# AOADMM-DataFusionFramework/Matlab-Code

Hardware: AMD Instinct MI355X
Metric: AO-ADMM outer iters/sec (+ mode-1 MTTKRP GFLOP/s), 2000^3 rank-20 CP (higher is better)
Workload: dtype f32

## Files before the change

matlab-code_amd/csrc/contract.hip:

```cpp
#include "contract.h"
#include "device_utils.h"
#include "small_dev.h"

#include <algorithm>
#include <cstdlib>

namespace aoadmm {

typedef float f32x4 __attribute__((ext_vector_type(4)));
typedef double f64x2 __attribute__((ext_vector_type(2)));
typedef double f64x4 __attribute__((ext_vector_type(4)));

static constexpr int kTileRows = 128;
static constexpr int kGroup = 8;

struct KArgs {
  const void* X;
  const void* frag;
  void* T;
  int64_t tiles_per_batch, ntiles, batch_stride, M, ld, C, Cg, trows;
  int groups_per_chunk, R;
  int flush_every;
};

typedef float f32x2 __attribute__((ext_vector_type(2)));

__global__ void pack_frag16_f32(const double* __restrict__ F, int64_t ldF, int64_t C, int R, int NT, int EX,
                                int64_t Cg, float* __restrict__ frag) {
  const int64_t idx = (int64_t)blockIdx.x * blockDim.x + threadIdx.x;
  const int64_t nmain = (int64_t)NT * Cg * 128;
  if (idx < nmain) {
    const int kk = idx & 1;
    const int lane = (idx >> 1) & 63;
    const int64_t g = (idx >> 7) % Cg;
    const int nt = (int)((idx >> 7) / Cg);
    const int64_t c = 8 * g + 4 * kk + (lane >> 4);
    const int r = 16 * nt + (lane & 15);
    frag[idx] = (c < C && r < R) ? (float)F[c + ldF * r] : 0.f;
  } else if (EX && idx < nmain + Cg * 32) {
    const int64_t j = idx - nmain;
    const int e = j & 3, q = (j >> 2) & 3, kk = (j >> 4) & 1;
    const int64_t g = j >> 5;
    const int64_t c = 8 * g + 4 * kk + q;
    const int r = 16 * NT + e;
    frag[idx] = (c < C && r < R) ? (float)F[c + ldF * r] : 0.f;
  }
}

__device__ __forceinline__ float quarter_sum4(float a, float b, float c, float d) {
  const auto ab = __builtin_amdgcn_permlane16_swap(__float_as_uint(a), __float_as_uint(b), false, false);
  const auto cd = __builtin_amdgcn_permlane16_swap(__float_as_uint(c), __float_as_uint(d), false, false);
  const float s_ab = __uint_as_float(ab[0]) + __uint_as_float(ab[1]);
  const float s_cd = __uint_as_float(cd[0]) + __uint_as_float(cd[1]);
  const auto x = __builtin_amdgcn_permlane32_swap(__float_as_uint(s_ab), __float_as_uint(s_cd), false, false);
  return __uint_as_float(x[0]) + __uint_as_float(x[1]);
}

constexpr int kFlushEvery = 3;
template <int NT, bool EX, bool L2 = false>
__global__ __launch_bounds__(256, NT <= 2 ? 2 : 1) void contract16_f32(KArgs a) {
  static_assert(!L2 || NT == 1, "two-level accumulation exists for one 16-column tile (R <= 20)");
  const int lane = threadIdx.x & 63;
  const int64_t wt = (int64_t)blockIdx.x * 4 + (threadIdx.x >> 6);
  if (wt >= a.ntiles) return;
  const int chunk = blockIdx.y;
  const int64_t b = wt / a.tiles_per_batch;
  const int64_t m0 = (wt - b * a.tiles_per_batch) * kTileRows;
  const int r16 = lane & 15, q = lane >> 4;
  int64_t row0 = m0 + 4 * r16, row1 = m0 + 64 + 4 * r16;
  if (row0 >= a.M) row0 = m0;
  if (row1 >= a.M) row1 = m0;
  const int64_t g0 = (int64_t)chunk * a.groups_per_chunk;
  int64_t g1 = g0 + a.groups_per_chunk;
  if (g1 > a.Cg) g1 = a.Cg;
  const int64_t gfull = (a.C / kGroup < g1) ? a.C / kGroup : g1;
  const float* X = reinterpret_cast<const float*>(a.X) + b * a.batch_stride;
  const float* xp0 = X + row0 + (kGroup * g0 + q) * a.ld;
  const float* xp1 = X + row1 + (kGroup * g0 + q) * a.ld;
  const int64_t ld4 = 4 * a.ld;
  const f32x2* fp = reinterpret_cast<const f32x2*>(a.frag) + g0 * 64 + lane;
  const int64_t fnt = a.Cg * 64;
  const f32x4* fe = reinterpret_cast<const f32x4*>(reinterpret_cast<const f32x2*>(a.frag) + (int64_t)NT * a.Cg * 64) + g0 * 8 + q;

  f32x4 acc[NT][2][4];
  f32x2 accE[2][4][2];
#define AO_PKFMA_LO(ACC, X2, E2) asm("v_pk_fma_f32 %0, %1, %2, %0 op_sel:[0,0,0] op_sel_hi:[0,1,1]" : "+v"(ACC) : "v"(X2), "v"(E2));
#define AO_PKFMA_HI(ACC, X2, E2) asm("v_pk_fma_f32 %0, %1, %2, %0 op_sel:[1,0,0] op_sel_hi:[1,1,1]" : "+v"(ACC) : "v"(X2), "v"(E2));
#pragma unroll
  for (int h = 0; h < 2; ++h)
#pragma unroll
    for (int v = 0; v < 4; ++v) {
      accE[h][v][0] = f32x2{0.f, 0.f};
      accE[h][v][1] = f32x2{0.f, 0.f};
#pragma unroll
      for (int nt = 0; nt < NT; ++nt) acc[nt][h][v] = f32x4{0.f, 0.f, 0.f, 0.f};
    }

  extern __shared__ __attribute__((aligned(16))) float t_lds[];
  double* l2 = reinterpret_cast<double*>(t_lds) + (threadIdx.x >> 6) * 2048 + lane;
  double accE2[2][4];
  if (L2) {
#pragma unroll
    for (int k = 0; k < 32; ++k) l2[k * 64] = 0.0;
#pragma unroll
    for (int h = 0; h < 2; ++h)
#pragma unroll
      for (int v = 0; v < 4; ++v) accE2[h][v] = 0.0;
  }
#define AO_FLUSH()                                                                                   \
  {                                                                                                  \
    _Pragma("unroll") for (int h = 0; h < 2; ++h) {                                                  \
      _Pragma("unroll") for (int vb = 0; vb < 4; vb += 2) {                                          \
        _Pragma("unroll") for (int v = vb; v < vb + 2; ++v)                                          \
          _Pragma("unroll") for (int i = 0; i < 4; ++i) {                                            \
            l2[((h * 4 + v) * 4 + i) * 64] += (double)acc[0][h][v][i];                               \
            acc[0][h][v][i] = 0.f;                                                                   \
          }                                                                                          \
        __builtin_amdgcn_sched_barrier(0);                                                           \
      }                                                                                              \
    }                                                                                                \
    if (EX) {       \
      _Pragma("unroll") for (int h = 0; h < 2; ++h)                                                  \
        _Pragma("unroll") for (int v = 0; v < 4; ++v) {                                              \
          accE2[h][v] += (double)quarter_sum4(accE[h][v][0][0], accE[h][v][0][1], accE[h][v][1][0], accE[h][v][1][1]); \
          accE[h][v][0] = f32x2{0.f, 0.f};                                                           \
          accE[h][v][1] = f32x2{0.f, 0.f};                                                           \
        }                                                                                            \
    }                                                                                                \
  }
  f32x4 x0[4], x1[4], x2[4], e0[2], e1[2], e2[2];
  f32x2 f0[NT], f1[NT], f2[NT];
  const int64_t ng = gfull > g0 ? gfull - g0 : 0;
  const int64_t gstep = kGroup * a.ld;
#define AO_LOAD1(XS, GI, S)                                                                          \
  XS[S] = __builtin_nontemporal_load(reinterpret_cast<const f32x4*>((((S) & 1) ? xp1 : xp0) + (GI) * gstep + ((S) >> 1) * ld4));
#define AO_LOADF(FS, ES, GI)                                                                         \
  {                                                                                                  \
    _Pragma("unroll") for (int nt = 0; nt < NT; ++nt) FS[nt] = fp[(GI) * 64 + nt * fnt];            \
    if (EX) { ES[0] = fe[(GI) * 8]; ES[1] = fe[(GI) * 8 + 4]; }                                      \
  }
#define AO_LOAD_STAGE(XS, FS, ES, GI)                                                                \
  { AO_LOAD1(XS, GI, 0) AO_LOAD1(XS, GI, 1) AO_LOAD1(XS, GI, 2) AO_LOAD1(XS, GI, 3) AO_LOADF(FS, ES, GI) }
#define AO_FMA_S(XS, FS, ES, S)                                                                      \
  {                                                                                                  \
    _Pragma("unroll") for (int v = 0; v < 4; ++v) {                                                  \
      _Pragma("unroll") for (int nt = 0; nt < NT; ++nt)                                              \
        acc[nt][(S) & 1][v] = __builtin_amdgcn_mfma_f32_16x16x4f32(XS[S][v], FS[nt][(S) >> 1], acc[nt][(S) & 1][v], 0, 0, 0); \
    }                                                                                                \
    if (EX) {       \
      const f32x2 xlo_ = __builtin_shufflevector(XS[S], XS[S], 0, 1), xhi_ = __builtin_shufflevector(XS[S], XS[S], 2, 3); \
      const f32x2 ea_ = __builtin_shufflevector(ES[(S) >> 1], ES[(S) >> 1], 0, 1);                   \
      const f32x2 eb_ = __builtin_shufflevector(ES[(S) >> 1], ES[(S) >> 1], 2, 3);                   \
      AO_PKFMA_LO(accE[(S) & 1][0][0], xlo_, ea_) AO_PKFMA_LO(accE[(S) & 1][0][1], xlo_, eb_)        \
      AO_PKFMA_HI(accE[(S) & 1][1][0], xlo_, ea_) AO_PKFMA_HI(accE[(S) & 1][1][1], xlo_, eb_)        \
      AO_PKFMA_LO(accE[(S) & 1][2][0], xhi_, ea_) AO_PKFMA_LO(accE[(S) & 1][2][1], xhi_, eb_)        \
      AO_PKFMA_HI(accE[(S) & 1][3][0], xhi_, ea_) AO_PKFMA_HI(accE[(S) & 1][3][1], xhi_, eb_)        \
    }                                                                                                \
  }
// ... 746 lines not shown
    return;
  }
  AO_REQUIRE(prec == AOADMM_PREC_F32 || prec == AOADMM_PREC_F64, "bad precision id %d", prec);
  AO_REQUIRE(pl.tprec == prec, "contraction plan and tensor precision disagree");
  if (pl.lead) {
    AO_REQUIRE(prec == AOADMM_PREC_F32, "leading-mode contraction exists for fp32 tensors only");
    launch_contract_lead(X, pl, F, ldF, frag_ws, T, s, ev0, ev1);
    return;
  }
  const int64_t Cg = cdiv(pl.C, kGroup);
  KArgs a;
  a.X = X; a.frag = frag_ws; a.T = T;
  a.tiles_per_batch = cdiv(pl.M, tile_rows(prec));
  a.ntiles = pl.nbatch * a.tiles_per_batch;
  a.batch_stride = pl.batch_stride; a.M = pl.M; a.ld = pl.ld; a.C = pl.C; a.Cg = Cg;
  a.trows = pl.trows();
  a.groups_per_chunk = (int)cdiv(Cg, pl.nchunk);
  a.R = pl.R;
  AO_REQUIRE(a.ntiles > 0 && pl.C > 0, "empty contraction");
  dim3 grid((unsigned)cdiv(a.ntiles, 4), (unsigned)pl.nchunk);
  AO_REQUIRE(cdiv(a.ntiles, 4) < (int64_t)2147483647, "tensor too large for one launch");
  if (prec == AOADMM_PREC_F32) {
    AO_REQUIRE(pl.ld % 4 == 0 && pl.M % 4 == 0 && pl.batch_stride % 4 == 0, "f32 layout must be padded to 4");
    const int rem = pl.R % 16;
    const bool ex = pl.R > 16 && rem >= 1 && rem <= 4;
    const int nt16 = ex ? pl.R / 16 : (pl.R + 15) / 16;
    const int64_t total = (int64_t)nt16 * Cg * 128 + (ex ? Cg * 32 : 0);
    pack_frag16_f32<<<(unsigned)cdiv(total, 256), 256, 0, s>>>(F, ldF, pl.C, pl.R, nt16, ex ? 1 : 0, Cg, (float*)frag_ws);
    AO_KERNEL_CHECK();
    size_t tsh = (size_t)4 * kTileRows * pl.R * sizeof(float);
    a.flush_every = kFlushEvery;
    if (nt16 == 1) tsh = (size_t)4 * 16384;
#define AO_GO(K) { if (tsh > 65536) ensure_dynamic_lds(reinterpret_cast<const void*>(K), (int)tsh); if (ev0) AO_HIP(hipEventRecord(ev0, s)); K<<<grid, 256, tsh, s>>>(a); }
    if (nt16 == 1 && !ex) AO_GO((contract16_f32<1, false, true>))
    else if (nt16 == 1) AO_GO((contract16_f32<1, true, true>))
    else if (nt16 == 2 && !ex) AO_GO((contract16_f32<2, false>))
    else if (nt16 == 2) AO_GO((contract16_f32<2, true>))
    else if (nt16 == 3 && !ex) AO_GO((contract16_f32<3, false>))
    else if (nt16 == 3) AO_GO((contract16_f32<3, true>))
    else if (nt16 == 4) AO_GO((contract16_f32<4, false>))
    else throw Error(AOADMM_ERR_UNSUPPORTED, "rank > 64 not supported");
#undef AO_GO
  } else {
    AO_REQUIRE(pl.ld % 2 == 0 && pl.M % 2 == 0 && pl.batch_stride % 2 == 0, "f64 layout must be padded to 2");
    const int rem = pl.R % 16;
    const bool ex = pl.R > 16 && rem >= 1 && rem <= 4;
    const int nt16 = ex ? pl.R / 16 : (pl.R + 15) / 16;
    const int64_t total = (int64_t)nt16 * Cg * 128 + (ex ? Cg * 32 : 0);
    pack_frag_f64<<<(unsigned)cdiv(total, 256), 256, 0, s>>>(F, ldF, pl.C, pl.R, nt16, ex ? 1 : 0, Cg, (double*)frag_ws);
    AO_KERNEL_CHECK();
    const size_t tsh = (size_t)4 * kTileRows64 * pl.R * sizeof(double);
#define AO_GO(K) { if (tsh > 65536) ensure_dynamic_lds(reinterpret_cast<const void*>(K), (int)tsh); if (ev0) AO_HIP(hipEventRecord(ev0, s)); K<<<grid, 256, tsh, s>>>(a); }
    if (nt16 == 1 && !ex) AO_GO((contract_f64<1, false>))
    else if (nt16 == 1) AO_GO((contract_f64<1, true>))
    else if (nt16 == 2 && !ex) AO_GO((contract_f64<2, false>))
    else if (nt16 == 2) AO_GO((contract_f64<2, true>))
    else if (nt16 == 3 && !ex) AO_GO((contract_f64<3, false>))
    else if (nt16 == 3) AO_GO((contract_f64<3, true>))
    else if (nt16 == 4) AO_GO((contract_f64<4, false>))
    else throw Error(AOADMM_ERR_UNSUPPORTED, "rank > 64 not supported");
#undef AO_GO
  }
  if (ev1) AO_HIP(hipEventRecord(ev1, s));
  AO_KERNEL_CHECK();
}

__global__ void factor_rowmajor_k(const double* __restrict__ F, int64_t ldF, int64_t rows, int R,
                                  double* __restrict__ Ft) {
  const int64_t idx = (int64_t)blockIdx.x * blockDim.x + threadIdx.x;
  if (idx >= rows * R) return;
  const int r = (int)(idx / rows);
  const int64_t a = idx - (int64_t)r * rows;
  Ft[a * R + r] = F[a + ldF * r];
}
static void factor_rowmajor(const double* F, int64_t ldF, int64_t rows, int R, double* Ft, hipStream_t s) {
  factor_rowmajor_k<<<(unsigned)cdiv(rows * R, 256), 256, 0, s>>>(F, ldF, rows, R, Ft);
  AO_KERNEL_CHECK();
}

template <typename TT, int VEC> struct TVec;
template <> struct TVec<float, 4> { typedef float type __attribute__((ext_vector_type(4))); };
template <> struct TVec<float, 1> { typedef float type; };
template <> struct TVec<double, 2> { typedef double type __attribute__((ext_vector_type(2))); };
template <> struct TVec<double, 1> { typedef double type; };
template <typename TT, int VEC>
__device__ __forceinline__ void fma_vec(double (&acc)[VEC], const TT* __restrict__ tp, const double* __restrict__ fp) {
  typedef typename TVec<TT, VEC>::type V;
  const V tv = __builtin_nontemporal_load(reinterpret_cast<const V*>(tp));
  if constexpr (VEC == 1) {
    acc[0] += (double)tv * fp[0];
  } else {
#pragma unroll
    for (int v = 0; v < VEC; ++v) acc[v] += (double)tv[v] * fp[v];
  }
}

template <typename TT, int VEC>
struct RVec {
  typename TVec<TT, VEC>::type t;
  double f[VEC];
  __device__ __forceinline__ void load(const TT* __restrict__ tp, const double* __restrict__ fp) {
    t = __builtin_nontemporal_load(reinterpret_cast<const typename TVec<TT, VEC>::type*>(tp));
#pragma unroll
    for (int v = 0; v < VEC; ++v) f[v] = fp[v];
  }
  __device__ __forceinline__ void fma(double (&acc)[VEC]) const {
    if constexpr (VEC == 1) {
      acc[0] += (double)t * f[0];
    } else {
#pragma unroll
      for (int v = 0; v < VEC; ++v) acc[v] += (double)t[v] * f[v];
    }
  }
};

template <typename TT, int VEC>
__global__ void reduce_inner_k(const TT* __restrict__ T, int nchunk, int64_t trows, int64_t A, int64_t Apad, int R,
                               const double* __restrict__ FaT, double scale, double* __restrict__ out,
                               int64_t ldOut, int rowmajor, int has_sys, SysBuild sys) {
  extern __shared__ double sh[];
  if (has_sys && blockIdx.x == 0) { sys_build_rider(sys); return; }
  const int64_t b = (int64_t)blockIdx.x - has_sys;
  const int t = threadIdx.x;
  const int64_t n = A * R, step = (int64_t)blockDim.x * VEC;
  double s0[VEC], s1[VEC], s2[VEC], s3[VEC];
#pragma unroll
  for (int v = 0; v < VEC; ++v) { s0[v] = 0; s1[v] = 0; s2[v] = 0; s3[v] = 0; }
  for (int ch = 0; ch < nchunk; ++ch) {
    const TT* Tb = T + ((int64_t)ch * trows + Apad * b) * R;
    int64_t e = (int64_t)t * VEC;
    for (; e + 3 * step < n; e += 4 * step) {
      RVec<TT, VEC> q0, q1, q2, q3;
      q0.load(Tb + e, FaT + e);
      q1.load(Tb + e + step, FaT + e + step);
      q2.load(Tb + e + 2 * step, FaT + e + 2 * step);
      q3.load(Tb + e + 3 * step, FaT + e + 3 * step);
      __builtin_amdgcn_sched_barrier(0);
      q0.fma(s0); q1.fma(s1); q2.fma(s2); q3.fma(s3);
    }
    for (; e < n; e += step) fma_vec<TT, VEC>(s0, Tb + e, FaT + e);
  }
#pragma unroll
  for (int v = 0; v < VEC; ++v) sh[t * VEC + v] = (s0[v] + s1[v]) + (s2[v] + s3[v]);
  __syncthreads();
  if (t < R) {
    const int nA = blockDim.x * VEC / R;
    double tot = 0.0;
    for (int i = 0; i < nA; ++i) tot += sh[i * R + t];
    if (rowmajor) out[b * R + t] = scale * tot;
    else out[b + ldOut * t] = scale * tot;
  }
}

template <typename TT, int VEC>
__global__ void reduce_inner2_k(const TT* __restrict__ T, int nchunk, int64_t trows, int64_t A, int64_t Apad, int64_t B,
                                int R, const double* __restrict__ FaT, double scale, double* __restrict__ out,
                                int64_t ldOut, int rowmajor, int has_sys, SysBuild sys) {
  extern __shared__ double sh[];
  if (has_sys && blockIdx.x == 0) { sys_build_rider(sys); return; }
  const int64_t b0 = 2 * ((int64_t)blockIdx.x - has_sys);
  const bool two = b0 + 1 < B;
  const int64_t b1 = two ? b0 + 1 : b0;
  const int t = threadIdx.x;
  const int64_t n = A * R, step = (int64_t)blockDim.x * VEC;
  double a0[VEC], a1[VEC], c0[VEC], c1[VEC];
#pragma unroll
  for (int v = 0; v < VEC; ++v) { a0[v] = 0; a1[v] = 0; c0[v] = 0; c1[v] = 0; }
  for (int ch = 0; ch < nchunk; ++ch) {
    const TT* Ta = T + ((int64_t)ch * trows + Apad * b0) * R;
    const TT* Tc = T + ((int64_t)ch * trows + Apad * b1) * R;
    int64_t e = (int64_t)t * VEC;
    for (; e + step < n; e += 2 * step) {
      RVec<TT, VEC> q0, q1, p0, p1;
      q0.load(Ta + e, FaT + e);
      q1.load(Ta + e + step, FaT + e + step);
      p0.t = __builtin_nontemporal_load(reinterpret_cast<const typename TVec<TT, VEC>::type*>(Tc + e));
      p1.t = __builtin_nontemporal_load(reinterpret_cast<const typename TVec<TT, VEC>::type*>(Tc + e + step));
      __builtin_amdgcn_sched_barrier(0);
#pragma unroll
      for (int v = 0; v < VEC; ++v) { p0.f[v] = q0.f[v]; p1.f[v] = q1.f[v]; }
      q0.fma(a0); q1.fma(a1); p0.fma(c0); p1.fma(c1);
    }
    for (; e < n; e += step) {
      RVec<TT, VEC> q0, p0;
      q0.load(Ta + e, FaT + e);
      p0.t = __builtin_nontemporal_load(reinterpret_cast<const typename TVec<TT, VEC>::type*>(Tc + e));
#pragma unroll
      for (int v = 0; v < VEC; ++v) p0.f[v] = q0.f[v];
      q0.fma(a0); p0.fma(c0);
    }
  }
  const int nt = blockDim.x * VEC;
#pragma unroll
  for (int v = 0; v < VEC; ++v) { sh[t * VEC + v] = a0[v] + a1[v]; sh[nt + t * VEC + v] = c0[v] + c1[v]; }
  __syncthreads();
  if (t < 2 * R) {
    const int which = t / R, r = t % R;
    if (which == 0 || two) {
      const int nA = nt / R;
      double tot = 0.0;
      for (int i = 0; i < nA; ++i) tot += sh[which * nt + i * R + r];
      const int64_t b = which ? b1 : b0;
      if (rowmajor) out[b * R + r] = scale * tot;
      else out[b + ldOut * r] = scale * tot;
    }
  }
}

size_t reduce_factor_scratch_bytes(int64_t rows, int R) { return (size_t)rows * R * sizeof(double); }

template <typename TT, int VEC>
static void launch_inner_t(const void* T, int nchunk, int64_t trows, int64_t A, int64_t Apad, int64_t B, int R,
                           const double* FaT, double scale, double* out, int64_t ldOut, hipStream_t s, int rowmajor,
                           const SysBuild* sys) {
  const int hs = sys ? 1 : 0;
  const SysBuild sb = sys ? *sys : SysBuild();
  const int rq = R / VEC;
  int threads = 256 / rq * rq;
  if (threads < rq) threads = rq;
  if (threads * VEC < R) threads = (R + VEC - 1) / VEC;
  if (B >= 1024 && 2 * R <= threads) {
    reduce_inner2_k<TT, VEC><<<(unsigned)((B + 1) / 2 + hs), threads, (size_t)2 * threads * VEC * sizeof(double), s>>>(
        (const TT*)T, nchunk, trows, A, Apad, B, R, FaT, scale, out, ldOut, rowmajor, hs, sb);
    return;
  }
  reduce_inner_k<TT, VEC><<<(unsigned)(B + hs), threads, (size_t)threads * VEC * sizeof(double), s>>>(
      (const TT*)T, nchunk, trows, A, Apad, R, FaT, scale, out, ldOut, rowmajor, hs, sb);
}

static bool sys_can_ride(const SysBuild* sys, int threads_min = 64) {
  return sys != nullptr && sys->R >= 1 && sys->R <= kSysRiderMaxR && threads_min >= 64;
}

bool launch_reduce_inner(const void* T, int tprec, int nchunk, int64_t trows, int64_t A, int64_t Apad,
                         int64_t B, int R, const double* Fa, int64_t ldFa, double scale,
                         double* out, int64_t ldOut, double* ft_scratch, hipStream_t s, const double* FaT,
                         int rowmajor_out, const SysBuild* sys) {
  AO_REQUIRE((int64_t)B < 2147483647ll, "reduce_inner: too many output rows for one launch");
  {
    const int vec = tprec == AOADMM_PREC_F32 ? (R % 4 == 0 ? 4 : 1) : (R % 2 == 0 ? 2 : 1);
    const int rq = R / vec;
    int threads = 256 / rq * rq;
    if (threads < rq) threads = rq;
    if (threads * vec < R) threads = (R + vec - 1) / vec;
    if (!sys_can_ride(sys, threads)) sys = nullptr;
  }
  if (FaT) ft_scratch = const_cast<double*>(FaT);
  else factor_rowmajor(Fa, ldFa, A, R, ft_scratch, s);
  if (tprec == AOADMM_PREC_F32) {
    if (R % 4 == 0) launch_inner_t<float, 4>(T, nchunk, trows, A, Apad, B, R, ft_scratch, scale, out, ldOut, s, rowmajor_out, sys);
    else launch_inner_t<float, 1>(T, nchunk, trows, A, Apad, B, R, ft_scratch, scale, out, ldOut, s, rowmajor_out, sys);
  } else {
    if (R % 2 == 0) launch_inner_t<double, 2>(T, nchunk, trows, A, Apad, B, R, ft_scratch, scale, out, ldOut, s, rowmajor_out, sys);
    else launch_inner_t<double, 1>(T, nchunk, trows, A, Apad, B, R, ft_scratch, scale, out, ldOut, s, rowmajor_out, sys);
  }
  AO_KERNEL_CHECK();
  return sys != nullptr;
}

static void outer_geometry(int64_t A, int64_t B, int R, int vec, int& TA, int64_t& nblkA, int& SB) {
  const int rq = (R + vec - 1) / vec;
  TA = 256 / rq;
  if (TA < 1) TA = 1;
  nblkA = cdiv(A, TA);
  int64_t sb = cdiv(2048, nblkA);
  if (sb > 64) sb = 64;
  if (sb > B) sb = B;
  if (sb < 1) sb = 1;
  SB = (int)sb;
}
static int outer_vec(int tprec, int R) {
  if (tprec == AOADMM_PREC_F32) return R % 4 == 0 ? 4 : 1;
  return R % 2 == 0 ? 2 : 1;
}

size_t reduce_outer_scratch_bytes(int64_t A, int64_t B, int R) {
  size_t worst = 0;
  for (int vec : {1, 2, 4}) {
    int TA, SB; int64_t nb;
    outer_geometry(A, B, R, vec, TA, nb, SB);
    worst = std::max(worst, (size_t)SB * A * R * sizeof(double));
  }
  return worst;
}

template <typename TT, int VEC>
__global__ void reduce_outer_k(const TT* __restrict__ T, int nchunk, int64_t trows, int64_t A,
                               int64_t Apad, int64_t B, int R, int TA, const double* __restrict__ FbT,
                               double* __restrict__ part, int has_sys, SysBuild sys) {
  if (has_sys && blockIdx.x == 0) {
    if (blockIdx.y == 0) sys_build_rider(sys);
    return;
  }
  const int t = threadIdx.x;
  const int rq = R / VEC;
  const int al = t / rq, r = (t - al * rq) * VEC;
  const int64_t a = ((int64_t)blockIdx.x - has_sys) * TA + al;
  const int SB = gridDim.y, sb = blockIdx.y;
  const int64_t bper = (B + SB - 1) / SB;
  const int64_t b0 = sb * bper;
  int64_t b1 = b0 + bper;
  if (b1 > B) b1 = B;
  if (al >= TA || a >= A) return;
  const int64_t bs = Apad * R;
  double s0[VEC], s1[VEC], s2[VEC], s3[VEC];
#pragma unroll
  for (int v = 0; v < VEC; ++v) { s0[v] = 0; s1[v] = 0; s2[v] = 0; s3[v] = 0; }
  for (int ch = 0; ch < nchunk; ++ch) {
    const TT* Tc = T + (int64_t)ch * trows * R + a * R + r;
    const double* Fr = FbT + r;
    int64_t b = b0;
    for (; b + 3 < b1; b += 4) {
      RVec<TT, VEC> q0, q1, q2, q3;
      q0.load(Tc + bs * b, Fr + b * R);
      q1.load(Tc + bs * (b + 1), Fr + (b + 1) * R);
      q2.load(Tc + bs * (b + 2), Fr + (b + 2) * R);
      q3.load(Tc + bs * (b + 3), Fr + (b + 3) * R);
      __builtin_amdgcn_sched_barrier(0);
      q0.fma(s0); q1.fma(s1); q2.fma(s2); q3.fma(s3);
    }
    for (; b < b1; ++b) fma_vec<TT, VEC>(s0, Tc + bs * b, Fr + b * R);
  }
#pragma unroll
  for (int v = 0; v < VEC; ++v) part[((int64_t)sb * A + a) * R + r + v] = (s0[v] + s1[v]) + (s2[v] + s3[v]);
}

__global__ void reduce_outer_fin(const double* __restrict__ part, int SB, int64_t A, int R, double scale,
                                 double* __restrict__ out, int64_t ldOut, int rowmajor) {
  int64_t idx = (int64_t)blockIdx.x * blockDim.x + threadIdx.x;
  if (idx >= A * R) return;
  const int64_t a = idx / R;
  const int r = (int)(idx - a * R);
  double t0 = 0.0, t1 = 0.0;
  int s = 0;
  const int64_t ar = A * R;
  for (; s + 7 < SB; s += 8) {
    const double v0 = part[(int64_t)s * ar + idx], v1 = part[(int64_t)(s + 1) * ar + idx];
    const double v2 = part[(int64_t)(s + 2) * ar + idx], v3 = part[(int64_t)(s + 3) * ar + idx];
    const double v4 = part[(int64_t)(s + 4) * ar + idx], v5 = part[(int64_t)(s + 5) * ar + idx];
    const double v6 = part[(int64_t)(s + 6) * ar + idx], v7 = part[(int64_t)(s + 7) * ar + idx];
    t0 += v0; t1 += v1; t0 += v2; t1 += v3; t0 += v4; t1 += v5; t0 += v6; t1 += v7;
  }
  for (; s + 1 < SB; s += 2) {
    t0 += part[(int64_t)s * ar + idx];
    t1 += part[(int64_t)(s + 1) * ar + idx];
  }
  if (s < SB) t0 += part[(int64_t)s * ar + idx];
  if (rowmajor) out[idx] = scale * (t0 + t1);
  else out[a + ldOut * r] = scale * (t0 + t1);
}

template <typename TT, int VEC>
static void launch_outer_t(const void* T, int nchunk, int64_t trows, int64_t A, int64_t Apad, int64_t B, int R,
                           const double* FbT, double* scratch, int& SB, hipStream_t s, const SysBuild* sys) {
  int TA; int64_t nb;
  outer_geometry(A, B, R, VEC, TA, nb, SB);
  int threads = TA * (R / VEC);
  threads = (threads + 63) / 64 * 64;
  const int hs = sys ? 1 : 0;
  reduce_outer_k<TT, VEC><<<dim3((unsigned)(nb + hs), (unsigned)SB), threads, 0, s>>>((const TT*)T, nchunk, trows, A, Apad, B,
                                                                                    R, TA, FbT, scratch, hs, sys ? *sys : SysBuild());
}

bool launch_reduce_outer(const void* T, int tprec, int nchunk, int64_t trows, int64_t A, int64_t Apad,
                         int64_t B, int R, const double* Fb, int64_t ldFb, double scale,
                         double* out, int64_t ldOut, double* scratch, double* ft_scratch, hipStream_t s,
                         const double* FbT, int rowmajor_out, const SysBuild* sys) {
  if (!sys_can_ride(sys)) sys = nullptr;
  if (FbT) ft_scratch = const_cast<double*>(FbT);
  else factor_rowmajor(Fb, ldFb, B, R, ft_scratch, s);
  int SB = 1;
  const int vec = outer_vec(tprec, R);
  if (tprec == AOADMM_PREC_F32) {
    if (vec == 4) launch_outer_t<float, 4>(T, nchunk, trows, A, Apad, B, R, ft_scratch, scratch, SB, s, sys);
    else launch_outer_t<float, 1>(T, nchunk, trows, A, Apad, B, R, ft_scratch, scratch, SB, s, sys);
  } else {
    if (vec == 2) launch_outer_t<double, 2>(T, nchunk, trows, A, Apad, B, R, ft_scratch, scratch, SB, s, sys);
    else launch_outer_t<double, 1>(T, nchunk, trows, A, Apad, B, R, ft_scratch, scratch, SB, s, sys);
  }
  AO_KERNEL_CHECK();
  reduce_outer_fin<<<(unsigned)cdiv(A * R, 256), 256, 0, s>>>(scratch, SB, A, R, scale, out, ldOut, rowmajor_out);
  AO_KERNEL_CHECK();
  return sys != nullptr;
}

template <typename TT, int RMAX>
__global__ __launch_bounds__(256) void small_mttkrp_k(SmallMttkrp a, int has_sys, SysBuild sys) {
  extern __shared__ double sf[];
  if (has_sys && blockIdx.x == 0) { sys_build_rider(sys); return; }
  const int row = (int)blockIdx.x - has_sys;
  const int R = a.R, Na = a.Na, Nb = a.Nb;
  double* fa = sf;
  double* fb = sf + (size_t)Na * R;
  double* red = fb + (size_t)(Nb > 0 ? Nb : 1) * R;
  for (int e = threadIdx.x; e < Na * R; e += 256) { const int i = e / R, r = e - i * R; fa[e] = a.Fa[i + a.lda * r]; }
  for (int e = threadIdx.x; e < Nb * R; e += 256) { const int i = e / R, r = e - i * R; fb[e] = a.Fb ? a.Fb[i + a.ldb * r] : 1.0; }
  __syncthreads();
  const TT* X = reinterpret_cast<const TT*>(a.X) + (int64_t)row * a.sn;
  double acc[RMAX];
#pragma unroll
  for (int r = 0; r < RMAX; ++r) acc[r] = 0.0;
  const int npairs = Na * Nb;
  for (int p = threadIdx.x; p < npairs; p += 256) {
    const int ia = p % Na, ib = p / Na;
    const double x = (double)X[(int64_t)ia * a.sa + (int64_t)ib * a.sb];
#pragma unroll
    for (int r = 0; r < RMAX; ++r)
      if (r < R) acc[r] += x * (fa[ia * R + r] * fb[ib * R + r]);
  }
  const int lane = threadIdx.x & 63, w = threadIdx.x >> 6;
#pragma unroll
  for (int r = 0; r < RMAX; ++r) {
    const double v = wave_sum(acc[r]);
    if (lane == 0) red[w * RMAX + r] = v;
  }
  __syncthreads();
  if ((int)threadIdx.x < R) {
    const int r = threadIdx.x;
    const double tot = (red[r] + red[RMAX + r]) + (red[2 * RMAX + r] + red[3 * RMAX + r]);
    a.out[row + a.ldOut * r] = a.scale * tot;
  }
}

bool small_mttkrp_ok(int64_t elems, int nd, const int64_t* dims, int R) {
  const bool off = getenv("AOADMM_NO_SMALL_MTTKRP") != nullptr;
  if (off || elems > kSmallMttkrpElems || !(nd == 2 || nd == 3) || R > 16) return false;
  int64_t sum = 0;
  for (int i = 0; i < nd; ++i) sum += dims[i];
  return (size_t)(sum * R + 64) * sizeof(double) <= 40 * 1024;
}

bool small_mttkrp(const SmallMttkrp& a, int prec, int64_t rows, hipStream_t s, const SysBuild* sys) {
  if (!sys_can_ride(sys)) sys = nullptr;
  const int hs = sys ? 1 : 0;
  const SysBuild sb = sys ? *sys : SysBuild();
  AO_REQUIRE(a.R >= 1 && a.R <= 16 && rows >= 1 && a.Na >= 1 && a.Nb >= 1, "small_mttkrp: bad sizes");
  const int rmax = a.R <= 4 ? 4 : (a.R <= 8 ? 8 : 16);
  const size_t lds = ((size_t)(a.Na + a.Nb) * a.R + 4 * rmax) * sizeof(double);
  AO_REQUIRE(lds <= 48 * 1024, "small_mttkrp: factors do not fit LDS");
#define AO_SM(TT, RM) small_mttkrp_k<TT, RM><<<(unsigned)(rows + hs), 256, lds, s>>>(a, hs, sb)
  if (prec == AOADMM_PREC_F32) { if (rmax == 4) AO_SM(float, 4); else if (rmax == 8) AO_SM(float, 8); else AO_SM(float, 16); }
  else { if (rmax == 4) AO_SM(double, 4); else if (rmax == 8) AO_SM(double, 8); else AO_SM(double, 16); }
#undef AO_SM
  AO_KERNEL_CHECK();
  return sys != nullptr;
}

template <typename TT>
__global__ void t_to_colmajor_k(const TT* __restrict__ T, int nchunk, int64_t trows, int64_t A, int R,
                                double scale, double* __restrict__ out, int64_t ldOut) {
  int64_t idx = (int64_t)blockIdx.x * blockDim.x + threadIdx.x;
  if (idx >= A * R) return;
  const int64_t a = idx / R;
  const int r = (int)(idx - a * R);
  double tot = 0.0;
  for (int ch = 0; ch < nchunk; ++ch) tot += (double)T[(int64_t)ch * trows * R + idx];
  out[a + ldOut * r] = scale * tot;
}

void launch_t_to_colmajor(const void* T, int tprec, int nchunk, int64_t trows, int64_t A, int R, double scale,
                          double* out, int64_t ldOut, hipStream_t s) {
  const unsigned nb = (unsigned)cdiv(A * R, 256);
  if (tprec == AOADMM_PREC_F32) t_to_colmajor_k<float><<<nb, 256, 0, s>>>((const float*)T, nchunk, trows, A, R, scale, out, ldOut);
  else t_to_colmajor_k<double><<<nb, 256, 0, s>>>((const double*)T, nchunk, trows, A, R, scale, out, ldOut);
  AO_KERNEL_CHECK();
}

}
```

Baseline: 127.6.

## Generalize inner reduction to NB rows and retile outer reduction with thread groups

The inner reduction kernel now processes NB=4 output rows per block instead of 2, sharing each factor-row load across more T rows, and is chosen based on CU count. The outer reduction is reworked: fixed 256-thread blocks hold multiple B-range groups reduced through LDS, two A rows are handled per thread, and the split count is sized from occupancy-derived resident blocks. The aim is more factor reuse and better bandwidth use in the partial contractions, at the cost of extra registers, LDS and occupancy queries on the host.

```diff
diff --git a/matlab-code_amd/csrc/contract.hip b/matlab-code_amd/csrc/contract.hip
--- a/matlab-code_amd/csrc/contract.hip
+++ b/matlab-code_amd/csrc/contract.hip
@@ -4,6 +4,7 @@
 
 #include <algorithm>
 #include <cstdlib>
+#include <mutex>
 
 namespace aoadmm {
 
@@ -1056,59 +1057,85 @@
   }
 }
 
-template <typename TT, int VEC>
-__global__ void reduce_inner2_k(const TT* __restrict__ T, int nchunk, int64_t trows, int64_t A, int64_t Apad, int64_t B,
-                                int R, const double* __restrict__ FaT, double scale, double* __restrict__ out,
-                                int64_t ldOut, int rowmajor, int has_sys, SysBuild sys) {
+template <typename TT, int VEC, int NB>
+__global__ void reduce_innerN_k(const TT* __restrict__ T, int nchunk, int64_t trows, int64_t A,
+                                int64_t Apad, int64_t B, int R, const double* __restrict__ FaT, double scale,
+                                double* __restrict__ out, int64_t ldOut, int rowmajor, int has_sys, SysBuild sys) {
+  typedef typename TVec<TT, VEC>::type V;
   extern __shared__ double sh[];
   if (has_sys && blockIdx.x == 0) { sys_build_rider(sys); return; }
-  const int64_t b0 = 2 * ((int64_t)blockIdx.x - has_sys);
-  const bool two = b0 + 1 < B;
-  const int64_t b1 = two ? b0 + 1 : b0;
+  const int64_t bf = NB * ((int64_t)blockIdx.x - has_sys);
   const int t = threadIdx.x;
   const int64_t n = A * R, step = (int64_t)blockDim.x * VEC;
-  double a0[VEC], a1[VEC], c0[VEC], c1[VEC];
-#pragma unroll
-  for (int v = 0; v < VEC; ++v) { a0[v] = 0; a1[v] = 0; c0[v] = 0; c1[v] = 0; }
+  double acc[NB][VEC];
+#pragma unroll
+  for (int j = 0; j < NB; ++j)
+#pragma unroll
+    for (int v = 0; v < VEC; ++v) acc[j][v] = 0;
   for (int ch = 0; ch < nchunk; ++ch) {
-    const TT* Ta = T + ((int64_t)ch * trows + Apad * b0) * R;
-    const TT* Tc = T + ((int64_t)ch * trows + Apad * b1) * R;
+    const TT* Tb[NB];
+#pragma unroll
+    for (int j = 0; j < NB; ++j) Tb[j] = T + ((int64_t)ch * trows + Apad * (bf + j < B ? bf + j : B - 1)) * R;
     int64_t e = (int64_t)t * VEC;
     for (; e + step < n; e += 2 * step) {
-      RVec<TT, VEC> q0, q1, p0, p1;
-      q0.load(Ta + e, FaT + e);
-      q1.load(Ta + e + step, FaT + e + step);
-      p0.t = __builtin_nontemporal_load(reinterpret_cast<const typename TVec<TT, VEC>::type*>(Tc + e));
-      p1.t = __builtin_nontemporal_load(reinterpret_cast<const typename TVec<TT, VEC>::type*>(Tc + e + step));
+      RVec<TT, VEC> q0[NB], q1[NB];
+      q0[0].load(Tb[0] + e, FaT + e);
+      q1[0].load(Tb[0] + e + step, FaT + e + step);
+#pragma unroll
+      for (int j = 1; j < NB; ++j) {
+        q0[j].t = __builtin_nontemporal_load(reinterpret_cast<const V*>(Tb[j] + e));
+        q1[j].t = __builtin_nontemporal_load(reinterpret_cast<const V*>(Tb[j] + e + step));
+      }
       __builtin_amdgcn_sched_barrier(0);
 #pragma unroll
-      for (int v = 0; v < VEC; ++v) { p0.f[v] = q0.f[v]; p1.f[v] = q1.f[v]; }
-      q0.fma(a0); q1.fma(a1); p0.fma(c0); p1.fma(c1);
+      for (int j = 1; j < NB; ++j)
+#pragma unroll
+        for (int v = 0; v < VEC; ++v) { q0[j].f[v] = q0[0].f[v]; q1[j].f[v] = q1[0].f[v]; }
+#pragma unroll
+      for (int j = 0; j < NB; ++j) { q0[j].fma(acc[j]); q1[j].fma(acc[j]); }
     }
     for (; e < n; e += step) {
-      RVec<TT, VEC> q0, p0;
-      q0.load(Ta + e, FaT + e);
-      p0.t = __builtin_nontemporal_load(reinterpret_cast<const typename TVec<TT, VEC>::type*>(Tc + e));
-#pragma unroll
-      for (int v = 0; v < VEC; ++v) p0.f[v] = q0.f[v];
-      q0.fma(a0); p0.fma(c0);
+      RVec<TT, VEC> q0[NB];
+      q0[0].load(Tb[0] + e, FaT + e);
+#pragma unroll
+      for (int j = 1; j < NB; ++j) q0[j].t = __builtin_nontemporal_load(reinterpret_cast<const V*>(Tb[j] + e));
+#pragma unroll
+      for (int j = 1; j < NB; ++j)
+#pragma unroll
+        for (int v = 0; v < VEC; ++v) q0[j].f[v] = q0[0].f[v];
+#pragma unroll
+      for (int j = 0; j < NB; ++j) q0[j].fma(acc[j]);
     }
   }
   const int nt = blockDim.x * VEC;
 #pragma unroll
-  for (int v = 0; v < VEC; ++v) { sh[t * VEC + v] = a0[v] + a1[v]; sh[nt + t * VEC + v] = c0[v] + c1[v]; }
+  for (int j = 0; j < NB; ++j)
+#pragma unroll
+    for (int v = 0; v < VEC; ++v) sh[j * nt + t * VEC + v] = acc[j][v];
   __syncthreads();
-  if (t < 2 * R) {
-    const int which = t / R, r = t % R;
-    if (which == 0 || two) {
-      const int nA = nt / R;
-      double tot = 0.0;
-      for (int i = 0; i < nA; ++i) tot += sh[which * nt + i * R + r];
-      const int64_t b = which ? b1 : b0;
-      if (rowmajor) out[b * R + r] = scale * tot;
-      else out[b + ldOut * r] = scale * tot;
-    }
-  }
+  for (int q = t; q < NB * R; q += blockDim.x) {
+    const int j = q / R, r = q - j * R;
+    const int64_t b = bf + j;
+    if (b >= B) continue;
+    const int nA = nt / R;
+    double tot = 0.0;
+    for (int i = 0; i < nA; ++i) tot += sh[j * nt + i * R + r];
+    if (rowmajor) out[b * R + r] = scale * tot;
+    else out[b + ldOut * r] = scale * tot;
+  }
+}
+
+static int device_cus() {
+  static std::mutex mu;
+  static int dev_of = -1, cus = 0;
+  std::lock_guard<std::mutex> lock(mu);
+  int dev = 0;
+  AO_HIP(hipGetDevice(&dev));
+  if (dev != dev_of) {
+    AO_HIP(hipDeviceGetAttribute(&cus, hipDeviceAttributeMultiprocessorCount, dev));
+    dev_of = dev;
+  }
+  return std::max(cus, 1);
 }
 
 size_t reduce_factor_scratch_bytes(int64_t rows, int R) { return (size_t)rows * R * sizeof(double); }
@@ -1123,8 +1150,9 @@
   int threads = 256 / rq * rq;
   if (threads < rq) threads = rq;
   if (threads * VEC < R) threads = (R + VEC - 1) / VEC;
-  if (B >= 1024 && 2 * R <= threads) {
-    reduce_inner2_k<TT, VEC><<<(unsigned)((B + 1) / 2 + hs), threads, (size_t)2 * threads * VEC * sizeof(double), s>>>(
+  constexpr int NB = 4;
+  if (cdiv(B, NB) >= device_cus()) {
+    reduce_innerN_k<TT, VEC, NB><<<(unsigned)(cdiv(B, NB) + hs), threads, (size_t)NB * threads * VEC * sizeof(double), s>>>(
         (const TT*)T, nchunk, trows, A, Apad, B, R, FaT, scale, out, ldOut, rowmajor, hs, sb);
     return;
   }
@@ -1162,71 +1190,148 @@
   return sys != nullptr;
 }
 
-static void outer_geometry(int64_t A, int64_t B, int R, int vec, int& TA, int64_t& nblkA, int& SB) {
+struct OuterGeom {
+  int TA;
+  int RPT;
+  int NG;
+  int64_t nblkA;
+  int SB;
+};
+constexpr int kOuterThreads = 256;
+constexpr int kOuterMinGroups = 4;
+constexpr int kOuterMinB = 8;
+static int64_t gcd64(int64_t a, int64_t b) { while (b) { const int64_t t = a % b; a = b; b = t; } return a; }
+static OuterGeom outer_geometry(int64_t A, int64_t B, int R, int vec, int esize, int64_t resident) {
+  OuterGeom g;
   const int rq = (R + vec - 1) / vec;
-  TA = 256 / rq;
-  if (TA < 1) TA = 1;
-  nblkA = cdiv(A, TA);
-  int64_t sb = cdiv(2048, nblkA);
-  if (sb > 64) sb = 64;
-  if (sb > B) sb = B;
-  if (sb < 1) sb = 1;
-  SB = (int)sb;
+  const int tmax = std::max(1, kOuterThreads / kOuterMinGroups / rq);
+  const int64_t whole = 128 / gcd64((int64_t)R * esize, 128);
+  int64_t ta = tmax;
+  if (whole <= tmax) ta = tmax / whole * whole;
+  if (ta > A) ta = whole <= tmax ? std::min<int64_t>(ta, (A + whole - 1) / whole * whole) : A;
+  g.TA = (int)std::max<int64_t>(ta, 1);
+  int64_t ng = kOuterThreads / ((int64_t)g.TA * rq);
+  ng = std::min<int64_t>(ng, std::max<int64_t>(B / kOuterMinB, 1));
+  g.NG = (int)std::max<int64_t>(std::min<int64_t>(ng, 16), 1);
+  g.RPT = A >= 2 * (int64_t)g.TA ? 2 : 1;
+  g.nblkA = cdiv(A, (int64_t)g.TA * g.RPT);
+  int64_t sb = resident / g.nblkA;
+  sb = std::min<int64_t>(sb, B / ((int64_t)kOuterMinB * g.NG));
+  g.SB = (int)std::max<int64_t>(std::min<int64_t>(sb, 64), 1);
+  return g;
 }
 static int outer_vec(int tprec, int R) {
   if (tprec == AOADMM_PREC_F32) return R % 4 == 0 ? 4 : 1;
   return R % 2 == 0 ? 2 : 1;
 }
 
-size_t reduce_outer_scratch_bytes(int64_t A, int64_t B, int R) {
-  size_t worst = 0;
-  for (int vec : {1, 2, 4}) {
-    int TA, SB; int64_t nb;
-    outer_geometry(A, B, R, vec, TA, nb, SB);
-    worst = std::max(worst, (size_t)SB * A * R * sizeof(double));
-  }
-  return worst;
-}
-
-template <typename TT, int VEC>
+template <typename TT, int VEC, int RPT>
 __global__ void reduce_outer_k(const TT* __restrict__ T, int nchunk, int64_t trows, int64_t A,
-                               int64_t Apad, int64_t B, int R, int TA, const double* __restrict__ FbT,
+                               int64_t Apad, int64_t B, int R, int TA, int NG, const double* __restrict__ FbT,
                                double* __restrict__ part, int has_sys, SysBuild sys) {
+  typedef typename TVec<TT, VEC>::type V;
+  extern __shared__ double sh[];
   if (has_sys && blockIdx.x == 0) {
     if (blockIdx.y == 0) sys_build_rider(sys);
     return;
   }
   const int t = threadIdx.x;
   const int rq = R / VEC;
-  const int al = t / rq, r = (t - al * rq) * VEC;
-  const int64_t a = ((int64_t)blockIdx.x - has_sys) * TA + al;
-  const int SB = gridDim.y, sb = blockIdx.y;
-  const int64_t bper = (B + SB - 1) / SB;
-  const int64_t b0 = sb * bper;
-  int64_t b1 = b0 + bper;
+  const int lg = TA * rq;
+  const int g = t / lg, l = t - g * lg;
+  const int al = l / rq, r = (l - al * rq) * VEC;
+  const int64_t a = ((int64_t)blockIdx.x - has_sys) * TA * RPT + al;
+  const int64_t nrange = (int64_t)gridDim.y * NG;
+  const int64_t bper = (B + nrange - 1) / nrange;
+  int64_t b0 = ((int64_t)blockIdx.y * NG + g) * bper, b1 = b0 + bper;
+  if (b0 > B) b0 = B;
   if (b1 > B) b1 = B;
-  if (al >= TA || a >= A) return;
   const int64_t bs = Apad * R;
-  double s0[VEC], s1[VEC], s2[VEC], s3[VEC];
-#pragma unroll
-  for (int v = 0; v < VEC; ++v) { s0[v] = 0; s1[v] = 0; s2[v] = 0; s3[v] = 0; }
-  for (int ch = 0; ch < nchunk; ++ch) {
-    const TT* Tc = T + (int64_t)ch * trows * R + a * R + r;
-    const double* Fr = FbT + r;
-    int64_t b = b0;
-    for (; b + 3 < b1; b += 4) {
-      RVec<TT, VEC> q0, q1, q2, q3;
-      q0.load(Tc + bs * b, Fr + b * R);
-      q1.load(Tc + bs * (b + 1), Fr + (b + 1) * R);
-      q2.load(Tc + bs * (b + 2), Fr + (b + 2) * R);
-      q3.load(Tc + bs * (b + 3), Fr + (b + 3) * R);
-      __builtin_amdgcn_sched_barrier(0);
-      q0.fma(s0); q1.fma(s1); q2.fma(s2); q3.fma(s3);
-    }
-    for (; b < b1; ++b) fma_vec<TT, VEC>(s0, Tc + bs * b, Fr + b * R);
-  }
-#pragma unroll
-  for (int v = 0; v < VEC; ++v) part[((int64_t)sb * A + a) * R + r + v] = (s0[v] + s1[v]) + (s2[v] + s3[v]);
+  constexpr int U = RPT == 1 ? 4 : 2;
+  double s[RPT][U][VEC];
+#pragma unroll
+  for (int j = 0; j < RPT; ++j)
+#pragma unroll
+    for (int u = 0; u < U; ++u)
+#pragma unroll
+      for (int v = 0; v < VEC; ++v) s[j][u][v] = 0;
+  if (g < NG && a < A) {
+    for (int ch = 0; ch < nchunk; ++ch) {
+      const TT* Tc[RPT];
+#pragma unroll
+      for (int j = 0; j < RPT; ++j) Tc[j] = T + ((int64_t)ch * trows + (a + (int64_t)j * TA < A ? a + (int64_t)j * TA : a)) * R + r;
+      const double* Fr = FbT + r;
+      int64_t b = b0;
+      for (; b + U - 1 < b1; b += U) {
+        RVec<TT, VEC> q[U][RPT];
+#pragma unroll
+        for (int u = 0; u < U; ++u) q[u][0].load(Tc[0] + bs * (b + u), Fr + (b + u) * R);
+#pragma unroll
+        for (int u = 0; u < U; ++u)
+#pragma unroll
+          for (int j = 1; j < RPT; ++j) q[u][j].t = __builtin_nontemporal_load(reinterpret_cast<const V*>(Tc[j] + bs * (b + u)));
+        __builtin_amdgcn_sched_barrier(0);
+#pragma unroll
+        for (int u = 0; u < U; ++u)
+#pragma unroll
+          for (int j = 0; j < RPT; ++j) {
+#pragma unroll
+            for (int v = 0; v < VEC; ++v) q[u][j].f[v] = q[u][0].f[v];
+            q[u][j].fma(s[j][u]);
+          }
+      }
+      for (; b < b1; ++b) {
+        RVec<TT, VEC> q[RPT];
+        q[0].load(Tc[0] + bs * b, Fr + b * R);
+#pragma unroll
+        for (int j = 1; j < RPT; ++j) q[j].t = __builtin_nontemporal_load(reinterpret_cast<const V*>(Tc[j] + bs * b));
+#pragma unroll
+        for (int j = 0; j < RPT; ++j) {
+#pragma unroll
+          for (int v = 0; v < VEC; ++v) q[j].f[v] = q[0].f[v];
+          q[j].fma(s[j][0]);
+        }
+      }
+    }
+  }
+  double tot[RPT][VEC];
+#pragma unroll
+  for (int j = 0; j < RPT; ++j)
+#pragma unroll
+    for (int v = 0; v < VEC; ++v) {
+      if constexpr (U == 4) tot[j][v] = (s[j][0][v] + s[j][1][v]) + (s[j][2][v] + s[j][3][v]);
+      else tot[j][v] = s[j][0][v] + s[j][1][v];
+    }
+  double* dst = part + ((int64_t)blockIdx.y * A + a) * R + r;
+  if (NG == 1) {
+#pragma unroll
+    for (int j = 0; j < RPT; ++j)
+      if (g < NG && a + (int64_t)j * TA < A) {
+#pragma unroll
+        for (int v = 0; v < VEC; ++v) dst[(int64_t)j * TA * R + v] = tot[j][v];
+      }
+    return;
+  }
+  const int gl = lg * RPT;
+  if (g < NG) {
+#pragma unroll
+    for (int j = 0; j < RPT; ++j)
+#pragma unroll
+      for (int v = 0; v < VEC; ++v) sh[((g * RPT + j) * lg + l) * VEC + v] = tot[j][v];
+  }
+  __syncthreads();
+  if (g == 0) {
+#pragma unroll
+    for (int j = 0; j < RPT; ++j)
+      if (a + (int64_t)j * TA < A) {
+#pragma unroll
+        for (int v = 0; v < VEC; ++v) {
+          double x = sh[(j * lg + l) * VEC + v];
+          for (int q = 1; q < NG; ++q) x += sh[(q * gl + j * lg + l) * VEC + v];
+          dst[(int64_t)j * TA * R + v] = x;
+        }
+      }
+  }
 }
 
 __global__ void reduce_outer_fin(const double* __restrict__ part, int SB, int64_t A, int R, double scale,
@@ -1255,15 +1360,47 @@
 }
 
 template <typename TT, int VEC>
+static int64_t outer_resident() {
+  static std::mutex mu;
+  static int dev_of = -1;
+  static int64_t blocks = 0;
+  std::lock_guard<std::mutex> lock(mu);
+  int dev = 0;
+  AO_HIP(hipGetDevice(&dev));
+  if (dev != dev_of) {
+    int per_cu = 0;
+    AO_HIP(hipOccupancyMaxActiveBlocksPerMultiprocessor(&per_cu, reduce_outer_k<TT, VEC, 2>, kOuterThreads,
+                                                        (size_t)2 * kOuterThreads * VEC * sizeof(double)));
+    blocks = (int64_t)std::max(per_cu, 1) * device_cus();
+    dev_of = dev;
+  }
+  return blocks;
+}
+static OuterGeom outer_geometry_of(int tprec, int64_t A, int64_t B, int R) {
+  const int vec = outer_vec(tprec, R);
+  if (tprec == AOADMM_PREC_F32)
+    return outer_geometry(A, B, R, vec, 4, vec == 4 ? outer_resident<float, 4>() : outer_resident<float, 1>());
+  return outer_geometry(A, B, R, vec, 8, vec == 2 ? outer_resident<double, 2>() : outer_resident<double, 1>());
+}
+
+size_t reduce_outer_scratch_bytes(int64_t A, int64_t B, int R) {
+  const int sb = std::max(outer_geometry_of(AOADMM_PREC_F32, A, B, R).SB, outer_geometry_of(AOADMM_PREC_F64, A, B, R).SB);
+  return (size_t)sb * A * R * sizeof(double);
+}
+
+template <typename TT, int VEC>
 static void launch_outer_t(const void* T, int nchunk, int64_t trows, int64_t A, int64_t Apad, int64_t B, int R,
-                           const double* FbT, double* scratch, int& SB, hipStream_t s, const SysBuild* sys) {
-  int TA; int64_t nb;
-  outer_geometry(A, B, R, VEC, TA, nb, SB);
-  int threads = TA * (R / VEC);
-  threads = (threads + 63) / 64 * 64;
+                           const double* FbT, double* scratch, const OuterGeom& g, hipStream_t s, const SysBuild* sys) {
   const int hs = sys ? 1 : 0;
-  reduce_outer_k<TT, VEC><<<dim3((unsigned)(nb + hs), (unsigned)SB), threads, 0, s>>>((const TT*)T, nchunk, trows, A, Apad, B,
-                                                                                    R, TA, FbT, scratch, hs, sys ? *sys : SysBuild());
+  const size_t lds = g.NG > 1 ? (size_t)g.NG * g.RPT * g.TA * R * sizeof(double) : 0;
+  const dim3 grid((unsigned)(g.nblkA + hs), (unsigned)g.SB);
+  const SysBuild sb = sys ? *sys : SysBuild();
+  if (g.RPT == 2)
+    reduce_outer_k<TT, VEC, 2><<<grid, kOuterThreads, lds, s>>>((const TT*)T, nchunk, trows, A, Apad, B, R, g.TA, g.NG, FbT,
+                                                                 scratch, hs, sb);
+  else
+    reduce_outer_k<TT, VEC, 1><<<grid, kOuterThreads, lds, s>>>((const TT*)T, nchunk, trows, A, Apad, B, R, g.TA, g.NG, FbT,
+                                                                 scratch, hs, sb);
 }
 
 bool launch_reduce_outer(const void* T, int tprec, int nchunk, int64_t trows, int64_t A, int64_t Apad,
@@ -1273,17 +1410,18 @@
   if (!sys_can_ride(sys)) sys = nullptr;
   if (FbT) ft_scratch = const_cast<double*>(FbT);
   else factor_rowmajor(Fb, ldFb, B, R, ft_scratch, s);
-  int SB = 1;
   const int vec = outer_vec(tprec, R);
+  const OuterGeom g = outer_geometry_of(tprec, A, B, R);
+  AO_REQUIRE(g.nblkA + 1 < 2147483647ll, "reduce_outer: too many rows for one launch");
   if (tprec == AOADMM_PREC_F32) {
-    if (vec == 4) launch_outer_t<float, 4>(T, nchunk, trows, A, Apad, B, R, ft_scratch, scratch, SB, s, sys);
-    else launch_outer_t<float, 1>(T, nchunk, trows, A, Apad, B, R, ft_scratch, scratch, SB, s, sys);
+    if (vec == 4) launch_outer_t<float, 4>(T, nchunk, trows, A, Apad, B, R, ft_scratch, scratch, g, s, sys);
+    else launch_outer_t<float, 1>(T, nchunk, trows, A, Apad, B, R, ft_scratch, scratch, g, s, sys);
   } else {
-    if (vec == 2) launch_outer_t<double, 2>(T, nchunk, trows, A, Apad, B, R, ft_scratch, scratch, SB, s, sys);
-    else launch_outer_t<double, 1>(T, nchunk, trows, A, Apad, B, R, ft_scratch, scratch, SB, s, sys);
+    if (vec == 2) launch_outer_t<double, 2>(T, nchunk, trows, A, Apad, B, R, ft_scratch, scratch, g, s, sys);
+    else launch_outer_t<double, 1>(T, nchunk, trows, A, Apad, B, R, ft_scratch, scratch, g, s, sys);
   }
   AO_KERNEL_CHECK();
-  reduce_outer_fin<<<(unsigned)cdiv(A * R, 256), 256, 0, s>>>(scratch, SB, A, R, scale, out, ldOut, rowmajor_out);
+  reduce_outer_fin<<<(unsigned)cdiv(A * R, 256), 256, 0, s>>>(scratch, g.SB, A, R, scale, out, ldOut, rowmajor_out);
   AO_KERNEL_CHECK();
   return sys != nullptr;
 }
```

Result: no change. 128.1, median of 6 (+0.4%).
